# 1mishra/cbc

Hardware: AMD Instinct MI355X
Metric: Mbases/s encoded (bit-exact) on synthetic 150 bp SAM (higher is better)
Workload: dtype u32; 1 GPU; cfg2: synthetic 150 bp SAM, 10000000 reads per GPU vs a 248956422 bp uniform-ACGT contig, block-parallel encode; reads_rank0=10000000, blocks_rank0=2442, block_reads=4096, lds_bytes_per_block=15264, payload_bytes_rank0=20710203, parallelism=one GPU, no collective

## Files before the change

### cbc_amd/csrc/cbc_encode_body.h

```cpp
#ifndef CBC_ENCODE_BODY_H
#define CBC_ENCODE_BODY_H

#include <stdint.h>
#include <type_traits>
#include "../../include/cbc_gpu.h"
#include "cbc_plan.h"

#ifndef CBC_PRIO_CODER
#define CBC_PRIO_CODER 3
#define CBC_PRIO_MODEL 0
#endif
#define CBC_REC_PACK_AT 56u
#define CBC_AWORD     26u
#define CBC_M26       ((1u << 26) - 1u)
#define CBC_M25       ((1u << 25) - 1u)
#define CBC_RESCALE   (1u << 20)
#define CBC_NVARCTX   0xffffu
#define CBC_NOMEMO    0xffffffffu
#define CBC_BLOOM_LOG2 13u
#define CBC_ROLE_FUSED 0u
#define CBC_ROLE_MODEL 1u
#define CBC_ROLE_CODER 2u

#define CBC_LT_MATCH   0u
#define CBC_LT_SAMEREF 8u
#define CBC_LT_CHARS   16u

#define CBC_LDS_RLEN    0u
#define CBC_LDS_SNPS    256u
#define CBC_LDS_INDELS  512u
#define CBC_LDS_RNKEY   768u
#define CBC_LDS_RNEXC   (768u + CBC_CAP_NAME)
#define CBC_LDS_BLOOM   (768u + 2u * CBC_CAP_NAME)
#define CBC_LDS_P0      (768u + 2u * CBC_CAP_NAME + CBC_BLOOM_WORDS)
#define CBC_LDS_BATCH   CBC_PLAN_TABLE_WORDS
#ifndef CBC_BATCH_MIN
#define CBC_BATCH_MIN   40u
#endif
#define CBC_LDS_CTL     (CBC_LDS_BATCH + CBC_BATCH_SLOTS * CBC_BATCH_WORDS)
#define CBC_LDS_RING    (CBC_LDS_CTL + 8u)
#define CBC_LDS_RUN     (CBC_LDS_RING + CBC_RING_WORDS)
#define CBC_LDS_FIXED   CBC_PLAN_LDS_FIXED_WORDS

#ifdef CBC_EMU_TRACE
extern "C" void cbc_emu_trace(uint32_t read, uint32_t lo, uint32_t cnt, uint32_t n);
#endif

enum {
    CBC_PC_CODE1, CBC_PC_CODE1_REM, CBC_PC_CODE1_REM_EXACT,
    CBC_PC_QUIET, CBC_PC_QUIET_REM, CBC_PC_QUIET_REM_EXACT,
    CBC_PC_KNOWN0, CBC_PC_KNOWN0_REM,
    CBC_PC_X3, CBC_PC_X3_EXIT, CBC_PC_X3_FB_SHIFT, CBC_PC_X3_FB_REM,
    CBC_PC_SR, CBC_PC_SR_EXIT, CBC_PC_SR_FB_SHIFT, CBC_PC_SR_FB_REM,
    CBC_PC_N
};
#if defined(CBC_PATH_COUNTS) && !defined(__HIP_DEVICE_COMPILE__)
extern "C" void cbc_path_count(uint32_t what, uint32_t read);
extern "C" void cbc_path_mute(int on);
#define CBC_COUNT(what, read) cbc_path_count((what), (read))
#define CBC_COUNT_IF(cond, what, read) do { if (cond) cbc_path_count((what), (read)); } while (0)
#define CBC_COUNT_MUTE(on) cbc_path_mute(on)
#else
#define CBC_COUNT(what, read) do {} while (0)
#define CBC_COUNT_IF(cond, what, read) do {} while (0)
#define CBC_COUNT_MUTE(on) do {} while (0)
#endif

struct cbc_enc_args {
    const cbc_read_rec   *recs;
    const uint8_t        *seq;
    const uint32_t       *tok;
    const uint8_t        *names;
    const cbc_block_desc *blocks;
    const uint8_t        *ref;
    uint8_t              *out;
    cbc_block_result     *results;
    uint64_t ref_bytes, out_bytes, seq_bytes, n_tok, n_recs;
    uint32_t n_blocks, cap_pos, cap_var, names_bytes;
};

#if defined(CBC_STAMP) && defined(__HIP_DEVICE_COMPILE__)
#define CBC_T0() do { unsigned long long t_; asm volatile("s_memtime %0\n\ts_waitcnt lgkmcnt(0)" : "=s"(t_) :: "memory"); E.t_last = t_; } while (0)
#define CBC_TS(k) do { unsigned long long t_; asm volatile("s_memtime %0\n\ts_waitcnt lgkmcnt(0)" : "=s"(t_) :: "memory"); E.t_sum[k] += t_ - E.t_last; E.t_last = t_; } while (0)
#define CBC_TSM(k) do { unsigned long long t_; asm volatile("s_memtime %0\n\ts_waitcnt lgkmcnt(0)" : "=s"(t_) :: "memory"); t_sum[k] += t_ - t_last; t_last = t_; } while (0)
#elif defined(CBC_MARKS) && defined(__HIP_DEVICE_COMPILE__)
#define CBC_TSM(k) asm volatile("; ==== CBC_MARK M" #k)
#define CBC_T0() asm volatile("; ==== CBC_MARK start")
#define CBC_TS(k) asm volatile("; ==== CBC_MARK " #k)
#else
#define CBC_T0() do {} while (0)
#define CBC_TS(k) do {} while (0)
#define CBC_TSM(k) do {} while (0)
#endif

CBC_FN bool cbc_le64(uint64_t a, uint64_t b)
{
    uint32_t ah = (uint32_t)(a >> 32), al = (uint32_t)a, bh = (uint32_t)(b >> 32), bl = (uint32_t)b;
    return (ah < bh) | ((ah == bh) & (al <= bl));
}
CBC_FN bool cbc_fits64(uint64_t off, uint64_t len, uint64_t total)
{
    return cbc_le64(off, total) && cbc_le64(len, total - off);
}
CBC_FN uint32_t cbc_avail32(uint64_t total, uint32_t off)
{
    uint64_t a = total - off;
    if (!cbc_le64((uint64_t)off, total)) return 0u;
    return (uint32_t)(a >> 32) ? 0xffffffffu : (uint32_t)a;
}
CBC_FN uint32_t cbc_basepair(uint32_t c)
{
    return c == 'A' ? 0u : c == 'C' ? 1u : c == 'G' ? 2u : c == 'T' ? 3u : 4u;
}

template <class W>
struct CbcWin {
    typedef typename W::V32 V32;
    V32 w;
    CBC_MFN void clear() { w = W::splat(0u); }
    CBC_MFN void shift(uint32_t d)
    {
        if (d == 0u) return;
        if (d >= 256u) { clear(); return; }
        const V32 ln = W::lane();
        const V32 src = ln + (d >> 5);
        const V32 lo = W::lane_gather(w, src), hi = W::lane_gather(w, src + 1u);
        w = W::select(ln < 8u, W::funnel_shr(hi, lo, d & 31u), W::splat(0u));
    }
    CBC_MFN uint32_t first(uint32_t p, uint32_t rl)
    {
        uint32_t out = rl + 2u;
        if (p >= rl) return out;
        const V32 ln = W::lane();
        const uint32_t pw = p >> 5;
        const V32 a = W::select(ln == pw, w & (0xffffffffu << (p & 31u)), W::select(ln > pw, w, W::splat(0u)));
        const uint64_t hb = W::ballot(a != 0u);
        if (hb) {
            const uint32_t hl = W::ctz64(hb);
            const uint32_t pos = hl * 32u + W::ctz64((uint64_t)W::readlane(a, hl));
            if (pos < rl) out = pos - p;
        }
        return out;
    }
    CBC_MFN void set(uint32_t k)
    {
        if (k < 256u) w = w | W::select(W::lane() == (k >> 5), W::splat(1u << (k & 31u)), W::splat(0u));
    }
};

template <class W>
CBC_FN typename W::V32 cbc_small_start(uint32_t ones)
{
    typedef typename W::V32 V32;
    typedef typename W::Mask Mask;
    const V32 ln = W::lane();
    V32 sm = W::select(ln < ones, W::splat(1u), W::splat(0u));
    V32 r = (ln - CBC_LT_CHARS) >> 3, c = (ln - CBC_LT_CHARS) & 7u;
    Mask inch = (ln >= CBC_LT_CHARS) & (r < 6u) & (c < 5u);
    V32 cv = W::select(c == 4u, W::splat(1u), W::select(c == r, W::splat(0u), W::splat(8u)));
    Mask bump = ((r == 0u) & ((c == 1u) | (c == 2u))) | ((r == 1u) & ((c == 0u) | (c == 3u))) |
                ((r == 2u) & ((c == 0u) | (c == 3u))) | ((r == 3u) & ((c == 1u) | (c == 2u)));
    cv = W::select(bump, cv + 8u, cv);
    return W::select(inch, cv, sm);
}

template <class W, class = void> struct CbcHasLaneN : std::false_type {};
template <class W> struct CbcHasLaneN<W, std::void_t<decltype(&W::set_lane2_uv), decltype(&W::set_lane3)>> : std::true_type {};

template <class W, bool GEN = false>
struct CbcEnc {
    typedef typename W::V32 V32;
    typedef typename W::Mask Mask;

    typedef typename W::Uv Uv;
    Uv l, rng;
    Uv lm1;
    Uv thr0;
    CBC_MFN void set_l_forms()
    {
        lm1 = W::uv_opaque(l - 1u);
        thr0 = ((l & (1u << 24)) | (1u << 25)) - l;
    }
    static CBC_MFN bool rem_flag2(Uv tl, Uv th)
    {
#ifndef CBC_REM_OR
        if constexpr (!GEN) return W::uv_ge(tl > th ? tl : th, 0xfc000000u);
#endif
        return W::uv_ge(tl | th, 0xfc000000u);
    }
    uint32_t scale3;
    uint32_t bitpos, flushed;
    uint32_t *ring;
    uint32_t *out32; uint32_t cap_words;
    uint32_t status, nsym, fail_read, cur_read;
    V32 q_lo, q_cnt, q_n; uint32_t q_len;
    uint32_t role, batch_i; uint32_t *batch, *ctl;
    V32 b_lo, b_hi, b_n, b_fl, b_fh; uint32_t b_len, b_pos, b_stop, b_flags, seen_last;
    uint64_t b_neq;
    V32 rec_a, rec_s; uint32_t rec_n;
#ifdef CBC_STAMP
    unsigned long long t_last, t_sum[16];
#endif

    V32 small;
    V32 fkey, fexc; uint32_t fcount;
    V32 hkey, hexc; uint32_t hc0, hc1, hc2, hc3, hn0, hn1, hn2, hn3;
    uint32_t *rlen_exc, *snps_exc, *indels_exc, *rname_key, *rname_exc, *pos_val, *pos_occ, *pos_pre, *pos_idx, *var_ev, *bloom, *p0ev;
    uint32_t *runs;
    uint32_t snps_n, indels_n;
    uint32_t rn_count, rn_cap;
    uint32_t *vtab;
    uint32_t *fsp_key, *fsp_exc; uint32_t fsp_count;
    uint32_t *pos_ov_val, *pos_ov_occ; uint32_t pos_lds_cap;
    uint32_t *palpha; uint32_t pa_n0, pa_n1, pa_n2, pa_n3;
    uint32_t pos_card, cap_pos;
    uint32_t nev, nev1, cap_var;
    V32 p0cnt; uint32_t p0over;
    uint32_t L0;

    uint32_t prevPos, prevM, prevChar, win_pos;
    CbcWin<W> win;

    CBC_MFN void fail(uint32_t st) { if (status == CBC_ST_OK) { status = st; fail_read = cur_read; } }

    CBC_MFN void start_coder(uint32_t *ring_, bool pulls)
    {
        status = CBC_ST_OK; nsym = 0; fail_read = 0; cur_read = 0;
        l = W::uv(0u); set_l_forms(); rng = W::uv(CBC_M26 + 1u); scale3 = 0u; bitpos = 0; flushed = 0;
        ring = ring_;
        q_lo = W::splat(0u); q_cnt = W::splat(0u); q_n = W::splat(0u); q_len = 0;
        if (pulls) { b_lo = W::splat(0u); b_hi = W::splat(0u); b_n = W::splat(1u); b_fl = W::splat(0u); b_fh = W::splat(0u); }
        b_len = 0; b_pos = 0; b_stop = 64u; b_flags = 0; seen_last = 0; b_neq = 0;
        rec_a = W::splat(0u); rec_s = W::splat(0u); rec_n = 0;
    }
    CBC_MFN void start_handoff(uint32_t role_, uint32_t *batch_, uint32_t *ctl_) { role = role_; batch_i = 0; batch = batch_; ctl = ctl_; }
    CBC_MFN void start_models()
    {
        fkey = W::splat(0u); fexc = W::splat(0u); fcount = 0;
        hkey = W::splat(0u); hexc = W::splat(0u);
        hc0 = hc1 = hc2 = hc3 = 0; hn0 = hn1 = hn2 = hn3 = 256u;
        p0cnt = W::splat(0u); p0over = 0;
        prevPos = 0; prevM = 0; prevChar = 0; win_pos = 0;
        win_clear();
    }
    CBC_MFN void code_int(uint32_t v)
    {
        regsparse_code(hkey, hexc, 0u, 8u, hc0, hn0, 256u, 1u, v >> 24, CBC_ST_ASSERT);
        regsparse_code(hkey, hexc, 8u, 8u, hc1, hn1, 256u, 1u, (v >> 16) & 0xffu, CBC_ST_ASSERT);
        regsparse_code(hkey, hexc, 16u, 8u, hc2, hn2, 256u, 1u, (v >> 8) & 0xffu, CBC_ST_ASSERT);
        regsparse_code(hkey, hexc, 24u, 8u, hc3, hn3, 256u, 1u, v & 0xffu, CBC_ST_ASSERT);
    }

    CBC_MFN void place(const V32 &val, const V32 &len, const V32 &off, const Mask &m)
    {
        const V32 aligned = val << (W::splat(32u) - len);
        const V32 sh = off & 31u, w = (off >> 5) & (CBC_RING_WORDS - 1u);
        const Mask on = m & (len != 0u);
        W::lds_or(ring, w, aligned >> sh, on);
        W::lds_or(ring, (w + 1u) & (CBC_RING_WORDS - 1u), aligned << (W::splat(32u) - sh), on & (sh != 0u));
    }
    CBC_MFN void flush_full()
    {
        const V32 ln = W::lane();
        while ((bitpos >> 5) - flushed >= 64u) {
            const V32 idx = (ln + flushed) & (CBC_RING_WORDS - 1u);
            const V32 wv = W::load32(ring, idx, W::all(), 0u);
            if (flushed + 64u <= cap_words) W::store32(out32, ln + flushed, W::bswap_v(wv), W::all());
            else fail(CBC_ST_OUT_FULL);
            W::store32(ring, idx, W::splat(0u), W::all());
            flushed += 64u;
        }
    }
    CBC_MFN void put(uint32_t v, uint32_t n)
    {
        if (n == 0) return;
        place(W::splat(v), W::splat(n), W::splat(bitpos), W::lane() == 0u);
        bitpos += n;
        flush_full();
    }
    CBC_MFN void put_run(uint32_t bit, uint32_t n)
    {
        uint32_t pat = bit ? 0xffffffffu : 0u;
        while (n >= 32u) { put(pat, 32u); n -= 32u; }
        if (n) put(pat >> (32u - n), n);
    }
    CBC_MFN void pack(const V32 &rec_a, const V32 &rec_k3, uint32_t m)
    {
        const V32 ln = W::lane();
        const Mask in = ln < m;
        const V32 k1 = rec_a >> 26, bits = (rec_a & CBC_M26) >> ((W::splat(26u) - k1) & 31u);
        const Mask act = in & (k1 != 0u);
        const V32 k3 = W::select(in, rec_k3, W::splat(0u));
        const V32 s_in = W::scan_incl_add(k3), s_ex = s_in - k3;
        const V32 mark = W::select(act, s_ex + 1u, W::splat(0u));
// ... 817 lines not shown
            const Mask isesc = W::lane_bit(esc);
            F.p_card = cardv;
            F.p_lo = W::select(isesc, zero, c_esc + (pre0 + lt) * 10u);
            F.p_cnt = W::select(isesc, c_esc, (occ0 + eqb) * 10u);
            W::store32(pos_occ, kv, occ0 + eqa, live & (kv != 0u) & !dxbad);
        }
        {
            uint32_t carry = 0;
            const uint32_t cb = W::uni(pos_card);
            for (uint32_t b = 0; b < cb; b += 64u) {
                const V32 i = ln + b; const Mask m = (i != 0u) & (i < pos_card);
                const V32 o = W::load32(pos_occ, i, m, 0u);
                const V32 inc = W::scan_incl_add(o);
                W::store32(pos_pre, i, inc - o + carry, i < pos_card);
                carry += W::readlane(inc, 63u);
            }
        }

        st = W::select(capflag, W::splat((uint32_t)CBC_ST_CAP_FLAG), st);
        st = W::select(cappos, W::splat((uint32_t)CBC_ST_CAP_POS), st);
        st = W::select(dxbad, W::splat((uint32_t)CBC_ST_ASSERT), st);
        st = W::select(rlbad, W::splat((uint32_t)CBC_ST_ASSERT), st);
        F.st = st; F.esc = esc;
        F.bad = W::ballot(live & (st != (uint32_t)CBC_ST_OK));
    }

    CBC_MFN void var_code_dense(uint32_t ctx, uint32_t sym)
    {
        V32 ln = W::lane();
        uint32_t *row = vtab + (uint64_t)ctx * L0;
        W::list_fence();
        V32 ev[4];
        for (uint32_t q = 0; q < 4u; q++) { V32 i = ln + 64u * q; ev[q] = W::load32_list(row, i, i < L0, 0u); }
        V32 alo = W::splat(0u), aall = W::splat(0u);
        uint32_t esym = 0;
        for (uint32_t q = 0; q < 4u; q++) {
            V32 i = ln + 64u * q;
            alo = alo + W::select(i < sym, ev[q], W::splat(0u));
            aall = aall + ev[q];
            if ((sym >> 6) == q) esym = W::readlane(ev[q], sym & 63u);
        }
        const uint32_t lo = sym + W::reduce_add(alo), n = L0 + W::reduce_add(aall);
        encode(lo, 1u + esym, n);
        W::append_list(row, sym, esym + 10u);
        if (n + 10u >= CBC_RESCALE) {
            W::list_fence();
            for (uint32_t q = 0; q < 4u; q++) {
                V32 i = ln + 64u * q;
                V32 e = W::load32_list(row, i, i < L0, 0u);
                W::store32_list(row, i, (e + 1u) >> 1, i < L0);
            }
        }
    }
    CBC_MFN void var_code(uint32_t ctx, uint32_t sym)
    {
        if (ctx >= CBC_NVARCTX || sym >= L0) { fail(CBC_ST_ASSERT); return; }
        if (GEN) { var_code_dense(ctx, sym); return; }
        V32 ln = W::lane();
        uint32_t cn = 0, clo = 0, ceq = 0;
        const uint32_t key = (ctx << 8) | sym, strand1 = ctx & 1u;
        const uint32_t p0class = (((ctx >> 1) & 0x7fu) == 0u && (ctx >> 8) != 255u) ? 1u : 0u;
        uint32_t to_global = p0class ^ 1u;
        const uint32_t bkt = strand1 * 8u + ((ctx >> 8) & 7u);
        uint32_t have = 0, half_word = 0;
        if (p0class) {
            const uint32_t d = ctx >> 8, key16 = (d << 8) | sym;
            const uint32_t *arr = p0ev + bkt * CBC_P0_BUCKET_WORDS;
            have = W::readlane(p0cnt, bkt);
            const uint32_t nw = (have + 1u) >> 1;
            const V32 w = W::load32(arr, ln, ln < nw, 0xffffffffu);
            if (have & 1u) half_word = W::readlane(w, have >> 1);
            const V32 e0 = w & 0xffffu, e1 = w >> 16;
            const V32 acc = W::select((e0 >> 8) == d, W::select((e0 & 0xffu) < sym, W::splat(1u + (1u << 10)), W::splat(1u)) +
                                                       W::select(e0 == key16, W::splat(1u << 20), W::splat(0u)), W::splat(0u)) +
                            W::select((e1 >> 8) == d, W::select((e1 & 0xffu) < sym, W::splat(1u + (1u << 10)), W::splat(1u)) +
                                                       W::select(e1 == key16, W::splat(1u << 20), W::splat(0u)), W::splat(0u));
            const uint32_t tot = W::reduce_add(acc);
            cn = tot & 1023u; clo = (tot >> 10) & 1023u; ceq = tot >> 20;
            if (have >= CBC_P0_CAP) to_global = 1u;
        }
        uint32_t h1 = 0, h2 = 0, bw1 = 0, bw2 = 0, bb1 = 0, bb2 = 0;
        if ((to_global | ((p0over >> bkt) & 1u)) != 0u) {
            h1 = (ctx * 0x9E3779B1u) >> (32u - CBC_BLOOM_LOG2); h2 = (ctx * 0x85EBCA6Bu + 0x27D4EB2Fu) >> (32u - CBC_BLOOM_LOG2);
            const V32 bwv = W::load32(bloom, W::select(ln == 0u, W::splat(h1 >> 5), W::splat(h2 >> 5)), ln < 2u, 0u);
            bw1 = W::readlane(bwv, 0u); bw2 = W::readlane(bwv, 1u);
            bb1 = 1u << (h1 & 31u); bb2 = 1u << (h2 & 31u);
            if ((bw1 & bb1) && (bw2 & bb2)) {
                W::list_fence();
                const uint32_t cnt_s = strand1 ? nev1 : nev, base_s = strand1 ? cap_var - nev1 : 0u;
                const uint32_t nb = W::uni(cnt_s);
                for (uint32_t b = 0; b < nb; b += 512u) {
                    V32 ev[8];
                    for (uint32_t q = 0; q < 8u; q++) { V32 i = ln + (b + 64u * q); ev[q] = W::load32_list(var_ev, i + base_s, i < cnt_s, 0xffffffffu); }
                    for (uint32_t q = 0; q < 8u; q++) {
                        const V32 e = ev[q];
                        const uint64_t bc = W::ballot((e >> 8) == ctx);
                        if (bc) {
                            cn += W::popc64(bc);
                            clo += W::popc64(W::ballot(((e >> 8) == ctx) & ((e & 0xffu) < sym)));
                            ceq += W::popc64(W::ballot(e == key));
                        }
                    }
                }
            }
        }
        encode(sym + 10u * clo, 1u + 10u * ceq, L0 + 10u * cn);
        if (!to_global) {
            uint32_t *arr = p0ev + bkt * CBC_P0_BUCKET_WORDS;
            const uint32_t k16 = ((ctx >> 8) << 8) | sym;
            if (have & 1u) W::write_uni(arr, have >> 1, (half_word & 0xffffu) | (k16 << 16));
            else W::write_uni(arr, have >> 1, 0xffff0000u | k16);
            p0cnt = W::select(ln == bkt, p0cnt + 1u, p0cnt);
            return;
        }
        if (nev + nev1 >= cap_var) { fail(CBC_ST_CAP_VAR); return; }
        if (p0class) p0over |= 1u << bkt;
        if (!((bw1 & bb1) && (bw2 & bb2))) {
            if ((h1 >> 5) == (h2 >> 5)) W::write_uni(bloom, h1 >> 5, bw1 | bb1 | bb2);
            else { W::write_uni(bloom, h1 >> 5, bw1 | bb1); W::write_uni(bloom, h2 >> 5, bw2 | bb2); }
        }
        if (strand1) { nev1++; W::append_list(var_ev, cap_var - nev1, key); }
        else { W::append_list(var_ev, nev, key); nev++; }
    }

    CBC_MFN void win_clear() { win.clear(); }
    CBC_MFN void win_shift(uint32_t d) { win.shift(d); }
    CBC_MFN uint32_t win_first(uint32_t p, uint32_t rl) { return win.first(p, rl); }
    CBC_MFN void win_set(uint32_t k) { win.set(k); }

    struct Prep { V32 hdr0, lo, cnt; uint64_t ord; };
    CBC_MFN void prep_group(Prep &P, uint64_t neq, const V32 &r_tok, const uint32_t *tokb, uint32_t n_tok_blk)
    {
        const V32 zero = W::splat(0u);
        const Mask im = W::lane_bit(neq);
        const V32 hdr0 = W::load32(tokb, r_tok, im & (r_tok < n_tok_blk), 0u);
        const V32 hdr1 = W::load32(tokb, r_tok + 1u, im & ((r_tok + 1u) < n_tok_blk), 0u);
        const V32 n_cig = hdr0 & 0xffffu, n_md = hdr0 >> 16;
        const Mask valid = im & ((r_tok + 2u + n_cig + n_md) <= n_tok_blk) & (n_md < 1024u) &
                           ((hdr1 & 0xffffu) < 1024u) & ((hdr1 >> 16) < 1024u);
        const Mask snp_only = hdr1 == 0u;
        const V32 symv = W::select(snp_only, n_md & 0xffu, zero);
        const bool counted = snps_n + 10u * W::popc64(neq) + 10u < CBC_RESCALE;
        V32 lo_base = zero, lo_extra = zero, cntv = zero, newv = zero;
        if (counted) {
            const Mask cm = valid & (symv < L0);
            uint64_t rem = W::ballot(cm);
            while (rem) {
                const uint32_t v = W::readlane(symv, W::ctz64(rem));
                const Mask mv = cm & (symv == v);
                const uint64_t m = W::ballot(mv);
                rem &= ~m;
                uint32_t lo0, cnt0;
                dense_lookup(snps_exc, v, lo0, cnt0);
                const V32 before = W::prefix_popc(m) * 10u;
                cntv = W::select(mv, before + cnt0, cntv);
                lo_base = W::select(mv, W::splat(lo0), lo_base);
// ... 192 lines not shown
                    uint32_t k = 0, cum = 0; bool more = true;
                    for (uint32_t o = 0; o <= n_cig && E.status == CBC_ST_OK; o++) {
                        uint32_t op, len;
                        if (o < n_cig) { uint32_t t = CBC_TOK(2u + o); op = t & 15u; len = t >> 4; }
                        else { op = 99u; len = 1u; }
                        if (op == CBC_OP_M) { Mc += len; continue; }
                        if (op == CBC_OP_STAR || (op == CBC_OP_S && o == 0u)) { E.fail(CBC_ST_UNSUPPORTED); break; }
                        if (op == CBC_OP_D) {
                            if (pass == 1)
                                for (uint32_t c = 0; c < len && E.status == CBC_ST_OK; c++) {
                                    uint32_t g = Mc - prevD;
                                    if (E.q_len >= 56u) E.drain();
                                    E.var_code((p << 1) | strand, g);
                                    p += g; prevD = Mc;
                                }
                            continue;
                        }
                        for (uint32_t c = 0; c < len && E.status == CBC_ST_OK; c++) {
                            if (E.q_len >= 56u) E.drain();
                            if ((op == CBC_OP_I || op == 99u) && more && pass == 2) {
                                uint32_t limit = (op == 99u) ? rl + 1u : Mc + ins;
                                more = false;
                                while (k < n_md && E.status == CBC_ST_OK) {
                                    uint32_t t = CBC_TOK(2u + n_cig + k);
                                    uint32_t g = t >> 8;
                                    if (cum + g >= limit) { cum++; more = true; break; }
                                    if (E.q_len >= 56u) E.drain();
                                    cum += g;
                                    CBC_SNP(g, t & 0xffu, cum, p);
                                    cum++; k++;
                                }
                            }
                            if (op == 99u) break;
                            if (pass == 3) {
                                uint32_t g = Mc - prevI;
                                uint32_t base = cbc_basepair(CBC_READ_BYTE(Mc + ins));
                                E.var_code((p << 1) | strand, g);
                                p += g;
                                E.small_code(CBC_LT_CHARS + 5u * 8u, 5u, 8u, base);
                                prevI = Mc;
                            }
                            ins++;
                        }
                    }
                }
            }
            CBC_TSM(13);
#undef CBC_SNP
#undef CBC_TOK
#undef CBC_READ_BYTE
    }
};

template <class W, uint32_t ROLE>
CBC_FN void cbc_encode_stream(const cbc_enc_args &A, uint32_t blk, uint32_t *lds)
{
    const uint32_t role = ROLE;
    typedef typename W::V32 V32;
    typedef typename W::Mask Mask;
    const V32 ln = W::lane();
    const cbc_block_desc *bd = A.blocks + blk;
    CbcEnc<W> E;

    const uint64_t rec_base = bd->rec_base, seq_base = bd->seq_base, tok_base = bd->tok_base;
    const uint64_t ref_off = bd->ref_off, out_off = bd->out_off;
    const uint32_t out_cap = bd->out_cap, n_reads = bd->n_reads, name_off = bd->name_off;
    const uint32_t L0 = bd->read_length, n_tok_blk = bd->n_tok;

    E.start_coder(lds + CBC_LDS_RING, true);
    E.start_handoff(role, lds + CBC_LDS_BATCH, lds + CBC_LDS_CTL);
    if (ROLE != CBC_ROLE_FUSED) {
        if (ROLE == CBC_ROLE_MODEL) { W::write_uni(E.ctl, 0u, 0u); W::write_uni(E.ctl, 1u, 0u); W::write_uni(E.ctl, 2u, 0u); W::write_uni(E.ctl, 3u, 0u); }
        W::barrier();
    }
    const uint32_t payload_cap = bd->reserved;
    E.out32 = (uint32_t *)(A.out + out_off);
    E.cap_words = payload_cap >> 2;
    E.var_ev = (uint32_t *)(A.out + out_off + payload_cap);
    E.cap_var = payload_cap <= out_cap ? (out_cap - payload_cap) >> 2 : 0u;
    bool args_ok = cbc_fits64(out_off, out_cap, A.out_bytes) && ((out_off & 3u) == 0) && ((payload_cap & 3u) == 0) &&
                   (payload_cap <= out_cap) &&
                   cbc_fits64(rec_base, n_reads, A.n_recs) && cbc_fits64(tok_base, n_tok_blk, A.n_tok) &&
                   (L0 >= 1u && L0 <= 256u) && (name_off < A.names_bytes);
    if (!args_ok) { E.cap_words = 0; E.fail(CBC_ST_ASSERT); }
    if (n_reads > CBC_MAX_BLOCK_READS) E.fail(CBC_ST_UNSUPPORTED);

    E.L0 = L0;
    E.rlen_exc = lds + CBC_LDS_RLEN; E.snps_exc = lds + CBC_LDS_SNPS; E.indels_exc = lds + CBC_LDS_INDELS;
    E.rname_key = lds + CBC_LDS_RNKEY; E.rname_exc = lds + CBC_LDS_RNEXC;
    E.bloom = lds + CBC_LDS_BLOOM; E.p0ev = lds + CBC_LDS_P0; E.runs = lds + CBC_LDS_RUN;
    E.pos_val = lds + CBC_LDS_FIXED; E.pos_occ = E.pos_val + A.cap_pos; E.pos_pre = E.pos_occ + A.cap_pos;
    E.fsp_key = E.fsp_exc = nullptr; E.fsp_count = 0; E.pos_ov_val = E.pos_ov_occ = nullptr; E.pos_lds_cap = 0xffffffc0u; E.palpha = nullptr;
    E.pos_idx = E.pos_pre + A.cap_pos;
    E.cap_pos = A.cap_pos;
    if (ROLE != CBC_ROLE_MODEL) {
        for (uint32_t b = 0; b < CBC_POS_IDX_WORDS; b += 64u) W::store32(E.pos_idx, ln + b, W::splat(0u), W::all());
        for (uint32_t b = 0; b < CBC_RING_WORDS; b += 64u) W::store32(E.ring, ln + b, W::splat(0u), W::all());
        for (uint32_t b = 0; b < 256u; b += 64u) W::store32(E.rlen_exc, ln + b, W::splat(0u), W::all());
        W::write_uni(E.pos_val, 0u, 0xffffffffu); W::write_uni(E.pos_occ, 0u, 0u); W::write_uni(E.pos_pre, 0u, 0u);
    }
    if (ROLE != CBC_ROLE_CODER) {
        for (uint32_t b = 0; b < 512u; b += 64u) W::store32(E.snps_exc, ln + b, W::splat(0u), W::all());
        for (uint32_t b = 0; b < CBC_BLOOM_WORDS; b += 64u) W::store32(E.bloom, ln + b, W::splat(0u), W::all());
    }
    E.snps_n = L0; E.indels_n = L0;
    E.rn_count = 0; E.rn_cap = CBC_CAP_NAME; E.vtab = nullptr;
    E.pos_card = 1u;
    E.nev = 0; E.nev1 = 0;
    E.start_models();
    E.small = cbc_small_start<W>(10u);

    const uint4 *recs4 = (const uint4 *)(A.recs + rec_base);
    const uint8_t *seqb = A.seq + seq_base;
    const uint32_t *tokb = A.tok + tok_base;
    const uint8_t *refb = A.ref + ref_off;
    const uint64_t seq_avail = cbc_le64(seq_base, A.seq_bytes) ? A.seq_bytes - seq_base : 0;
    const uint64_t ref_avail = cbc_le64(ref_off, A.ref_bytes) ? A.ref_bytes - ref_off : 0;
    const uint32_t seq_lim = cbc_avail32(seq_avail, 0u), ref_lim = cbc_avail32(ref_avail, 0u);
#ifdef CBC_STAMP
    for (int i = 0; i < 16; i++) E.t_sum[i] = 0;
    CBC_T0();
#endif

    auto gen_header = [&]() {
        for (uint32_t k = 0; k < 34u && E.status == CBC_ST_OK; k++) {
            uint32_t v = (k == 0u) ? L0 : (k == 33u) ? 8u : CBC_WELL_SEED;
            E.code_int(v);
            if ((k & 7u) == 7u) E.drain();
        }
    };
    auto gen_rname = [&]() {
        for (uint32_t q = 0; E.status == CBC_ST_OK; q++) {
            uint32_t ch = (name_off + q < A.names_bytes) ? W::read_uni8(A.names, name_off + q) : 0u;
            E.rname_code(E.prevChar, ch);
            if ((q & 31u) == 31u) E.drain();
            if (ch == 0u) break;
            E.prevChar = ch;
        }
    };
    auto gen_sentinel = [&]() {
        if (E.q_len >= 56u) E.drain();
        E.cur_read = n_reads;
        E.rname_code(E.prevChar, (uint32_t)'\n');
        E.rname_code((uint32_t)'\n', 0u);
    };
    auto match_group = [&](uint32_t cn, const V32 &r_pos, const V32 &r_fl, const V32 &r_seq) -> uint64_t {
        const V32 vrl = W::select(ln < cn, r_fl >> 16, W::splat(0u));
        const V32 ro = r_pos - 1u;
        const uint32_t nd = W::uni(W::readlane(W::scan_incl_max(vrl), 63u) >> 2);
        V32 acc = W::splat(0u);
        for (uint32_t c = 0; c < nd; c += 8u) {
            V32 sv[8], rv[8];
            for (uint32_t q = 0; q < 8u; q++) {
                const uint32_t b = (c + q) * 4u;
                const Mask m = vrl >= b + 4u;
                sv[q] = W::load32_bytes(seqb + b, r_seq, m);
                rv[q] = W::load32_bytes(refb + b, ro, m);
            }
            for (uint32_t q = 0; q < 8u; q++) acc = acc | (sv[q] ^ rv[q]);
        }
        {
            const V32 tail = vrl & 3u, lb = vrl - tail;
            const Mask m = tail != 0u;
            const V32 s = W::load32_bytes(seqb, r_seq + lb, m), r = W::load32_bytes(refb, ro + lb, m);
            acc = acc | ((s ^ r) & ((W::splat(1u) << (tail * 8u)) - 1u));
        }
        return W::ballot(acc != 0u);
    };
    auto load_group = [&](uint32_t c0, V32 &r_pos, V32 &r_fl, V32 &r_seq, V32 &r_tok, bool check) -> bool {
        W::load_rec(recs4, ln + c0, (ln + c0) < n_reads, r_pos, r_fl, r_seq, r_tok);
        if (!check) return true;
        V32 vrl = r_fl >> 16;
        Mask live = (ln + c0) < n_reads;
        Mask bad = live & ((vrl == 0u) | (vrl > CBC_MAX_READ_LEN) | (r_pos == 0u) |
                           ((r_seq + vrl + 4u) > seq_lim) | ((r_pos + vrl + 3u) > ref_lim) | (r_tok >= n_tok_blk));
        uint64_t bb = W::ballot(bad);
        if (bb) { E.cur_read = c0 + W::ctz64(bb); E.fail(CBC_ST_ASSERT); return false; }
        return true;
    };

    if (ROLE == CBC_ROLE_MODEL) {
        if (CBC_PRIO_MODEL) W::prio(CBC_PRIO_MODEL);
        if (E.status == CBC_ST_OK) { gen_header(); E.seg_end(); }
        for (uint32_t c0 = 0; c0 < n_reads && E.status == CBC_ST_OK; c0 += 64u) {
            V32 r_pos, r_fl, r_seq, r_tok;
            E.cur_read = c0;
            if (E.q_len) E.publish(0u);
            uint64_t neq;
            if (!E.wait_group(c0 >> 6, neq)) { E.fail(CBC_ST_ASSERT); break; }
            load_group(c0, r_pos, r_fl, r_seq, r_tok, false);
            CBC_TS(0);
            if (c0 == 0u) { gen_rname(); E.seg_end(); }
            typename CbcEnc<W>::Prep P;
            E.prep_group(P, neq, r_tok, tokb, n_tok_blk);
            CBC_TS(14);
            uint64_t todo = neq;
            V32 nx_seq = W::splat(0u), nx_tok = W::splat(0u);
            uint32_t nx_j = 64u;
            auto prefetch = [&](uint32_t jn) {
                const uint32_t so = W::readlane(r_seq, jn), to = W::readlane(r_tok, jn), nrl = W::readlane(r_fl, jn) >> 16;
                V32 bo = ln * 4u;
                nx_seq = W::load32_bytes(seqb + so, bo, bo < nrl);
                nx_tok = W::load32(tokb + to, ln, (ln + to) < n_tok_blk, 0u);
                nx_j = jn;
            };
            auto prefetch_if_general = [&](uint64_t rest) {
                if (rest) { const uint32_t jn = W::ctz64(rest); if (!((P.ord >> jn) & 1ull)) prefetch(jn); }
            };
            typename CbcEnc<W>::Run R;
            R.pk = W::splat(0u); R.ca = R.pk; R.cb = R.pk; R.rm = 0ull; R.s = 0u; R.counted = 0u;
            while (todo && E.status == CBC_ST_OK) {
                const uint32_t j = W::ctz64(todo);
                if ((P.ord >> j) & 1ull) {
                    if (!E.run_pass(R, P, todo, r_pos, r_fl, r_seq, r_tok, tokb, seqb)) { P.ord &= ~R.rm; continue; }
                    todo &= ~R.rm;
                    prefetch_if_general(todo);
                    CBC_TS(2);
                    for (uint64_t rr = R.rm; rr && E.status == CBC_ST_OK; rr &= rr - 1ull) {
                        const uint32_t jr = W::ctz64(rr);
                        E.cur_read = c0 + jr;
                        E.run_record(R, W::readlane(P.hdr0, jr) >> 16, W::readlane(P.lo, jr), W::readlane(P.cnt, jr));
                        E.seg_end_fits();
                        CBC_TS(1);
                        if (E.q_len >= CBC_BATCH_MIN) E.drain();
                    }
                    continue;
                }
                if (nx_j != j) prefetch(j);
                todo &= todo - 1ull;
                E.cur_read = c0 + j;
                const V32 seqv = nx_seq, tokv = nx_tok;
                prefetch_if_general(todo);
                const typename CbcEnc<W>::PrepRec pr = { W::readlane(P.lo, j), W::readlane(P.cnt, j) };
                E.edits(W::readlane(r_pos, j), W::readlane(r_fl, j), W::readlane(r_tok, j), seqv, tokv, tokb, n_tok_blk, pr);
                E.seg_end_fits();
                CBC_TS(1);
                if (E.q_len >= CBC_BATCH_MIN) E.drain();
            }
        }
        if (E.status == CBC_ST_OK) { gen_sentinel(); E.seg_end(); }
#if defined(CBC_STAMP) && defined(__HIP_DEVICE_COMPILE__)
        if (E.cap_var >= 64u) for (int i = 0; i < 16; i++) {
            W::write_uni(E.var_ev + E.cap_var - 32u, 2 * i, (uint32_t)E.t_sum[i]); W::write_uni(E.var_ev + E.cap_var - 32u, 2 * i + 1, (uint32_t)(E.t_sum[i] >> 32)); }
#endif
        E.publish(CBC_BF_LAST);
        return;
    }

    const bool fused = ROLE == CBC_ROLE_FUSED;
    if (!fused) W::prio(CBC_PRIO_CODER);
    uint64_t neq_ahead = 0;
    auto look_ahead = [&](uint32_t g0) {
        V32 a_pos, a_fl, a_seq, a_tok;
        const uint32_t an = n_reads - g0 < 64u ? n_reads - g0 : 64u;
        const uint32_t saved = E.cur_read;
        CBC_TS(9);
        const bool okg = load_group(g0, a_pos, a_fl, a_seq, a_tok, true);
        neq_ahead = okg ? match_group(an, a_pos, a_fl, a_seq) : 0ull;
        E.post_group(g0 >> 6, neq_ahead, okg ? 0u : 1u);
        CBC_TS(15);
        if (okg) E.cur_read = saved;
    };
    if (!fused && n_reads != 0u && E.status == CBC_ST_OK) look_ahead(0u);
    if (E.status == CBC_ST_OK) { if (fused) { gen_header(); E.seg_end(); } else E.seg_consume(); }
    for (uint32_t c0 = 0; c0 < n_reads && E.status == CBC_ST_OK; c0 += 64u) {
        V32 r_pos, r_fl, r_seq, r_tok;
        const uint32_t cn = n_reads - c0 < 64u ? n_reads - c0 : 64u;
        E.cur_read = c0;
        uint64_t neq;
        typename CbcEnc<W>::Prep P;
        typename CbcEnc<W>::Run R;
        R.pk = W::splat(0u); R.ca = R.pk; R.cb = R.pk; R.rm = 0ull; R.s = 0u; R.counted = 0u;
        if (fused) {
            if (!load_group(c0, r_pos, r_fl, r_seq, r_tok, true)) break;
            neq = match_group(cn, r_pos, r_fl, r_seq);
            E.prep_group(P, neq, r_tok, tokb, n_tok_blk);
        } else {
            neq = neq_ahead;
            if (c0 + 64u < n_reads) look_ahead(c0 + 64u);
            if (E.status != CBC_ST_OK) break;
            load_group(c0, r_pos, r_fl, r_seq, r_tok, false);
        }
        typename CbcEnc<W>::Fixed F;
        E.fixed_group(F, c0, cn, r_pos, r_fl, neq);
        const V32 rdv = ln + c0;
        const V32 sr_hi = rdv * 10u - 9u, sr_n = rdv * 10u + 2u;
        const V32 sr_fh = CBC_FRAC(sr_hi, sr_n);
        const V32 t_hi = rdv * 10u + 1u, t_n = rdv * 10u + 255u;
        const V32 t_fh = CBC_FRAC(t_hi, t_n);
        const V32 rl_hi = F.rl_lo + F.rl_cnt;
        const V32 rl_fl = CBC_FRAC(F.rl_lo, t_n), rl_fh = CBC_FRAC(rl_hi, t_n);
        const V32 p_n = (F.p_card - 1u) * 10u + rdv * 10u + 1u, p_hi = F.p_lo + F.p_cnt;
        const V32 p_fl = CBC_FRAC(F.p_lo, p_n), p_fh = CBC_FRAC(p_hi, p_n);
        const V32 fl_n = rdv * 8u + 65536u, fl_hi = F.fl_lo + F.fl_cnt;
        const V32 fl_fl = CBC_FRAC(F.fl_lo, fl_n), fl_fh = CBC_FRAC(fl_hi, fl_n);
        const V32 m_hi = F.m_lo + F.m_cnt;
        const V32 m_fl = CBC_FRAC(F.m_lo, F.m_n), m_fh = CBC_FRAC(m_hi, F.m_n);

#define CBC_LZ(expr) [&]() -> uint32_t { return (expr); }
        auto code_record = [&](uint32_t j, auto first, auto esc) {
            const uint32_t r = c0 + j;
            E.cur_read = r;
            E.room(8u);
            const uint32_t tn = 255u + 10u * r;
            if (decltype(first)::value) {
                E.encode(1u, 1u, 2u); E.drain_q();
                if (fused) { gen_rname(); E.seg_end(); } else E.seg_consume();
            }
            if (decltype(first)::value) {
                const uint32_t tf = W::readlane(t_fh, j);
                E.step_fixed_quiet(CBC_LZ(W::readlane(F.rl_lo, j)), CBC_LZ(W::readlane(rl_hi, j)), CBC_LZ(tn), W::readlane(rl_fl, j), W::readlane(rl_fh, j));
                E.step_known0(CBC_LZ(W::readlane(t_hi, j)), CBC_LZ(tn), tf);
                E.step_known0(CBC_LZ(W::readlane(t_hi, j)), CBC_LZ(tn), tf);
                E.step_known0(CBC_LZ(W::readlane(t_hi, j)), CBC_LZ(tn), tf);
            } else {
                E.step_sameref_rl0(CBC_LZ(W::readlane(sr_hi, j)), CBC_LZ(10u * r + 2u), W::readlane(sr_fh, j),
                                   CBC_LZ(W::readlane(F.rl_lo, j)), CBC_LZ(W::readlane(rl_hi, j)), CBC_LZ(tn), W::readlane(rl_fl, j), W::readlane(rl_fh, j));
                E.step_known0_x3(CBC_LZ(W::readlane(t_hi, j)), CBC_LZ(tn), W::readlane(t_fh, j));
            }
            E.step_fixed(CBC_LZ(W::readlane(F.p_lo, j)), CBC_LZ(W::readlane(p_hi, j)), CBC_LZ(W::readlane(p_n, j)), W::readlane(p_fl, j), W::readlane(p_fh, j));
            if (decltype(esc)::value == 1 || (decltype(esc)::value == 2 && ((F.esc >> j) & 1ull))) {
                const uint32_t card = W::readlane(F.p_card, j);
                E.pos_alpha(W::read_uni(E.pos_val, card), card);
                E.drain_q();
            }
            E.step_fixed(CBC_LZ(W::readlane(F.fl_lo, j)), CBC_LZ(W::readlane(fl_hi, j)), CBC_LZ(65536u + 8u * r), W::readlane(fl_fl, j), W::readlane(fl_fh, j));
            E.step_fixed(CBC_LZ(W::readlane(F.m_lo, j)), CBC_LZ(W::readlane(m_hi, j)), CBC_LZ(W::readlane(F.m_n, j)), W::readlane(m_fl, j), W::readlane(m_fh, j));
            if ((neq >> j) & 1ull) {
                if (fused) {
                    if (((P.ord >> j) & 1ull) && !((R.rm >> j) & 1ull) &&
                        !E.run_pass(R, P, neq & (~0ull << j), r_pos, r_fl, r_seq, r_tok, tokb, seqb)) P.ord &= ~R.rm;
                    if ((P.ord >> j) & 1ull) E.run_record(R, W::readlane(P.hdr0, j) >> 16, W::readlane(P.lo, j), W::readlane(P.cnt, j));
                    else {
                        const uint32_t so = W::readlane(r_seq, j), to = W::readlane(r_tok, j), flw = W::readlane(r_fl, j);
                        const V32 bo = ln * 4u;
                        const V32 seqv = W::load32_bytes(seqb + so, bo, bo < (flw >> 16));
                        const V32 tokv = W::load32(tokb + to, ln, (ln + to) < n_tok_blk, 0u);
                        const typename CbcEnc<W>::PrepRec pr = { W::readlane(P.lo, j), W::readlane(P.cnt, j) };
                        E.edits(W::readlane(r_pos, j), flw, to, seqv, tokv, tokb, n_tok_blk, pr);
                    }
                    E.seg_end();
                } else E.seg_consume();
            }
        };
#undef CBC_LZ
        uint32_t jn = cn;
        if (F.bad) { const uint32_t fb = W::ctz64(F.bad); if (fb < cn) jn = fb; }
        typedef std::integral_constant<int, 0> Plain; typedef std::integral_constant<int, 1> Esc; typedef std::integral_constant<int, 2> Look;
        uint32_t j = 0;
        if (c0 == 0u && jn != 0u) { code_record(0u, std::true_type(), Look()); j = 1u; }
        while (j < jn && E.status == CBC_ST_OK) {
            const uint64_t ahead = F.esc >> j;
            uint32_t run_end = ahead ? j + W::ctz64(ahead) : jn;
            if (run_end > jn) run_end = jn;
            for (; j < run_end && E.status == CBC_ST_OK; j++) code_record(j, std::false_type(), Plain());
            if (j < jn && E.status == CBC_ST_OK) { code_record(j, std::false_type(), Esc()); j++; }
        }
        if (jn < cn && E.status == CBC_ST_OK) { E.cur_read = c0 + jn; E.fail(W::readlane(F.st, jn)); }
    }
    uint32_t nbytes = 0;
    if (E.status == CBC_ST_OK) {
        E.cur_read = n_reads;
        if (n_reads) E.encode(10u * n_reads - 9u, 11u, 10u * n_reads + 2u);
        else E.encode(1u, 1u, 2u);
        E.drain_q();
        if (fused) { gen_sentinel(); E.seg_end(); } else E.seg_consume();
    }
    if (E.status == CBC_ST_OK) { E.flush_recs(); nbytes = E.finish(); }
    if (E.status != CBC_ST_OK) nbytes = 0;
    if (!fused && E.status != CBC_ST_OK) E.abort_groups();
    if (!fused) E.pull_rest();
#if defined(CBC_STAMP) && defined(__HIP_DEVICE_COMPILE__)
    if (payload_cap >= 128u) for (int i = 0; i < 16; i++) {
        W::write_uni(E.out32, 2 * i, (uint32_t)E.t_sum[i]); W::write_uni(E.out32, 2 * i + 1, (uint32_t)(E.t_sum[i] >> 32)); }
#endif
    V32 resv = W::select(ln == 0u, W::splat(nbytes), W::select(ln == 1u, W::splat(E.status),
               W::select(ln == 2u, W::splat(E.nsym), W::splat(E.fail_read))));
    W::store32((uint32_t *)(A.results + blk), ln, resv, ln < 4u);
}

#endif
```

### cbc_amd/csrc/cbc_gpu.hip

```cpp
#include <new>
#include <time.h>
#include <dlfcn.h>
#include <rccl/rccl.h>

#include "cbc_gpu_internal.h"
#include "cbc_wave_gpu.h"
#include "cbc_encode_body.h"
#include "cbc_decode_body.h"
#include "cbc_stream_body.h"
#include "cbc_long_body.h"
#include "cbc_covx_body.h"
#include "cbc_stats_aln_body.h"

static_assert(CbcHasLaneN<WaveGPU>::value, "WaveGPU must supply set_lane2_uv and set_lane3");

extern __shared__ uint32_t cbc_lds[];

static __device__ __forceinline__ void cbc_encode_block(const cbc_enc_args &A)
{
    uint32_t blk = blockIdx.x;
    if (blk >= A.n_blocks) return;
    const uint32_t wid = (uint32_t)__builtin_amdgcn_readfirstlane((int)(threadIdx.x >> 6));
    if (wid == 0u) cbc_encode_stream<WaveGPU, CBC_ROLE_MODEL>(A, blk, cbc_lds);
    else cbc_encode_stream<WaveGPU, CBC_ROLE_CODER>(A, blk, cbc_lds);
}

__global__ void __launch_bounds__(128) __attribute__((amdgpu_waves_per_eu(5)))
cbc_encode_blocks_kernel(cbc_enc_args A) { cbc_encode_block(A); }

__global__ void __launch_bounds__(128) __attribute__((amdgpu_waves_per_eu(6)))
cbc_encode_blocks_kernel_w6(cbc_enc_args A) { cbc_encode_block(A); }

__global__ void __launch_bounds__(64)
cbc_decode_blocks_kernel(cbc_dec_args A)
{
    uint32_t blk = blockIdx.x;
    if (blk >= A.n_blocks) return;
    cbc_decode_stream<WaveGPU>(A, blk, cbc_lds);
}

__global__ void __launch_bounds__(64)
cbc_decode_blocks_span_kernel(cbc_dec_args A, uint32_t smax)
{
    uint32_t blk = blockIdx.x;
    if (blk >= A.n_blocks) return;
    cbc_decode_stream<WaveGPU, true>(A, blk, cbc_lds, smax);
}

__global__ void __launch_bounds__(64)
cbc_decode_blocks_edits_kernel(cbc_dec_args A, uint32_t smax, cbc_dec_edits E)
{
    uint32_t blk = blockIdx.x;
    if (blk >= A.n_blocks) return;
    cbc_decode_stream<WaveGPU, true, true>(A, blk, cbc_lds, smax, &E);
}

__global__ void __launch_bounds__(64)
cbc_encode_whole_kernel(cbc_stream_args A)
{
    const uint32_t n_streams = A.per_segment ? A.n_segs : 1u;
    for (uint32_t s = blockIdx.x; s < n_streams; s += gridDim.x) {
        if (s != blockIdx.x) {
            uint4 *t = (uint4 *)(A.vtab + (uint64_t)blockIdx.x * CBC_VTAB_WORDS);
            for (uint64_t i = threadIdx.x; i < CBC_VTAB_WORDS / 4; i += 64) t[i] = make_uint4(0, 0, 0, 0);
            __threadfence();
        }
        cbc_encode_whole<WaveGPU>(A, s, blockIdx.x, cbc_lds);
    }
}

__global__ void __launch_bounds__(64)
cbc_decode_whole_kernel(cbc_dstream_args A) { cbc_decode_whole<WaveGPU>(A, cbc_lds); }

#ifndef CBC_LONG_ENC_WAVES
#define CBC_LONG_ENC_WAVES 8
#endif
__global__ void __launch_bounds__(192) __attribute__((amdgpu_waves_per_eu(CBC_LONG_ENC_WAVES)))
cbc_long_encode_kernel(cbc_long_args A)
{
    if (blockIdx.x >= A.n_blocks) return;
    const uint32_t wid = (uint32_t)__builtin_amdgcn_readfirstlane((int)(threadIdx.x >> 6));
    if (wid == 0u) cbc_long_encode<WaveGPU, CBC_ROLE_MODEL>(A, blockIdx.x, cbc_lds);
    else if (wid == 1u) cbc_long_encode<WaveGPU, CBC_ROLE_CODER>(A, blockIdx.x, cbc_lds);
    else cbc_long_encode<WaveGPU, CBC_ROLE_WALKER>(A, blockIdx.x, cbc_lds);
// ... 1861 lines not shown
```

Before: 240,600 Mbases/s.

## Add register-resident hot variant context for the most frequent var_code key

Adds a dedicated register-held count table (two V32 pairs of packed 16-bit counts per strand) for the single hottest variant context (L0+2), so var_code for that context skips the LDS p0 bucket search, bloom lookup and global scan. The counts are prefix-summed with a wave reduction to derive the cumulative frequency. It also adds host-side counters and extra timing slots for profiling. The cost is extra VGPR pressure in the encode kernel (w5 variant only by default), which could hurt occupancy, and it relies on coding matching the original model exactly.

```diff
diff --git a/cbc_amd/csrc/cbc_encode_body.h b/cbc_amd/csrc/cbc_encode_body.h
--- a/cbc_amd/csrc/cbc_encode_body.h
+++ b/cbc_amd/csrc/cbc_encode_body.h
@@ -66,6 +66,31 @@
 #define CBC_COUNT_MUTE(on) do {} while (0)
 #endif
 
+enum {
+    CBC_VC_CALLS, CBC_VC_P0,
+    CBC_VC_HOT,
+    CBC_VC_FULL,
+    CBC_VC_BLOOM,
+    CBC_VC_SCAN, CBC_VC_SCAN_P0,
+    CBC_VC_N
+};
+#if defined(CBC_VAR_COUNTS) && !defined(__HIP_DEVICE_COMPILE__)
+extern "C" void cbc_var_count(uint32_t what, uint32_t strand);
+extern "C" void cbc_var_block(uint32_t blk);
+extern "C" int cbc_var_hot_off(void);
+#define CBC_VCOUNT(what, strand) cbc_var_count((what), (strand))
+#define CBC_VBLOCK(blk) cbc_var_block(blk)
+#define CBC_VAR_HOT_OFF() (cbc_var_hot_off() != 0)
+#else
+#define CBC_VCOUNT(what, strand) do {} while (0)
+#define CBC_VBLOCK(blk) do {} while (0)
+#define CBC_VAR_HOT_OFF() false
+#endif
+
+#ifndef CBC_HOT_CTX
+#define CBC_HOT_CTX 1
+#endif
+
 struct cbc_enc_args {
     const cbc_read_rec   *recs;
     const uint8_t        *seq;
@@ -83,15 +108,22 @@
 #define CBC_T0() do { unsigned long long t_; asm volatile("s_memtime %0\n\ts_waitcnt lgkmcnt(0)" : "=s"(t_) :: "memory"); E.t_last = t_; } while (0)
 #define CBC_TS(k) do { unsigned long long t_; asm volatile("s_memtime %0\n\ts_waitcnt lgkmcnt(0)" : "=s"(t_) :: "memory"); E.t_sum[k] += t_ - E.t_last; E.t_last = t_; } while (0)
 #define CBC_TSM(k) do { unsigned long long t_; asm volatile("s_memtime %0\n\ts_waitcnt lgkmcnt(0)" : "=s"(t_) :: "memory"); t_sum[k] += t_ - t_last; t_last = t_; } while (0)
+#define CBC_TN0(v) unsigned long long v; asm volatile("s_memtime %0\n\ts_waitcnt lgkmcnt(0)" : "=s"(v) :: "memory")
+#define CBC_TN(v, k) do { unsigned long long t_; asm volatile("s_memtime %0\n\ts_waitcnt lgkmcnt(0)" : "=s"(t_) :: "memory"); t_sum[k] += t_ - v; } while (0)
 #elif defined(CBC_MARKS) && defined(__HIP_DEVICE_COMPILE__)
 #define CBC_TSM(k) asm volatile("; ==== CBC_MARK M" #k)
+#define CBC_TN0(v) asm volatile("; ==== CBC_MARK N0")
+#define CBC_TN(v, k) asm volatile("; ==== CBC_MARK N" #k)
 #define CBC_T0() asm volatile("; ==== CBC_MARK start")
 #define CBC_TS(k) asm volatile("; ==== CBC_MARK " #k)
 #else
 #define CBC_T0() do {} while (0)
 #define CBC_TS(k) do {} while (0)
 #define CBC_TSM(k) do {} while (0)
-#endif
+#define CBC_TN0(v) do {} while (0)
+#define CBC_TN(v, k) do {} while (0)
+#endif
+#define CBC_STAMP_SLOTS 18
 
 CBC_FN bool cbc_le64(uint64_t a, uint64_t b)
 {
@@ -167,8 +199,9 @@
 template <class W, class = void> struct CbcHasLaneN : std::false_type {};
 template <class W> struct CbcHasLaneN<W, std::void_t<decltype(&W::set_lane2_uv), decltype(&W::set_lane3)>> : std::true_type {};
 
-template <class W, bool GEN = false>
+template <class W, bool GEN = false, bool HOT = false>
 struct CbcEnc {
+    static_assert(!(GEN && HOT), "the hot var context belongs to the block kernels");
     typedef typename W::V32 V32;
     typedef typename W::Mask Mask;
 
@@ -199,7 +232,7 @@
     uint64_t b_neq;
     V32 rec_a, rec_s; uint32_t rec_n;
 #ifdef CBC_STAMP
-    unsigned long long t_last, t_sum[16];
+    unsigned long long t_last, t_sum[CBC_STAMP_SLOTS];
 #endif
 
     V32 small;
@@ -217,6 +250,7 @@
     uint32_t nev, nev1, cap_var;
     V32 p0cnt; uint32_t p0over;
     uint32_t L0;
+    V32 hot_a0, hot_b0, hot_a1, hot_b1; uint32_t hot_n0, hot_n1, hot_key;
 
     uint32_t prevPos, prevM, prevChar, win_pos;
     CbcWin<W> win;
@@ -240,6 +274,10 @@
         hkey = W::splat(0u); hexc = W::splat(0u);
         hc0 = hc1 = hc2 = hc3 = 0; hn0 = hn1 = hn2 = hn3 = 256u;
         p0cnt = W::splat(0u); p0over = 0;
+        if constexpr (HOT) {
+            hot_a0 = W::splat(0u); hot_b0 = W::splat(0u); hot_a1 = W::splat(0u); hot_b1 = W::splat(0u); hot_n0 = 0; hot_n1 = 0;
+            hot_key = (L0 + 2u <= 254u && !CBC_VAR_HOT_OFF()) ? (L0 + 2u) << 8 : 0xffffffffu;
+        }
         prevPos = 0; prevM = 0; prevChar = 0; win_pos = 0;
         win_clear();
     }
@@ -1163,10 +1201,39 @@
             }
         }
     }
+    CBC_MFN void hot_code(V32 &a, V32 &b, uint32_t &n, uint32_t sym)
+    {
+        if (n >= 0xfffeu) { fail(CBC_ST_ASSERT); return; }
+        const V32 ln = W::lane();
+        const uint32_t q = sym >> 6, r = sym & 63u;
+        const uint32_t w = (q & 2u) ? W::readlane(b, r) : W::readlane(a, r);
+        const uint32_t ceq = (w >> ((q & 1u) * 16u)) & 0xffffu;
+        const uint64_t m_all = (1ull << (16u * q)) - 1ull, m_low = (m_all << 16) | 0xffffull;
+        const Mask low = ln < r;
+        const V32 fa = a & W::select(low, W::splat((uint32_t)m_low), W::splat((uint32_t)m_all));
+        const V32 fb = b & W::select(low, W::splat((uint32_t)(m_low >> 32)), W::splat((uint32_t)(m_all >> 32)));
+        const uint32_t clo = W::reduce_add((fa & 0xffffu) + (fa >> 16) + (fb & 0xffffu) + (fb >> 16));
+        W::expect_eq((clo + ceq <= n && n < 0xffffu) ? 1u : 0u, 1u, "hot var context: a count above the use count");
+        encode(sym + 10u * clo, 1u + 10u * ceq, L0 + 10u * n);
+        const uint32_t inc = 1u << ((q & 1u) * 16u);
+        const Mask one = ln == r;
+        a = a + W::select(one, W::splat((q & 2u) ? 0u : inc), W::splat(0u));
+        b = b + W::select(one, W::splat((q & 2u) ? inc : 0u), W::splat(0u));
+        n++;
+    }
     CBC_MFN void var_code(uint32_t ctx, uint32_t sym)
     {
         if (ctx >= CBC_NVARCTX || sym >= L0) { fail(CBC_ST_ASSERT); return; }
         if (GEN) { var_code_dense(ctx, sym); return; }
+        CBC_VCOUNT(CBC_VC_CALLS, ctx & 1u);
+        if constexpr (HOT) {
+            if ((ctx & ~1u) == hot_key) {
+                CBC_VCOUNT(CBC_VC_P0, ctx & 1u); CBC_VCOUNT(CBC_VC_HOT, ctx & 1u);
+                if (ctx & 1u) hot_code(hot_a1, hot_b1, hot_n1, sym);
+                else hot_code(hot_a0, hot_b0, hot_n0, sym);
+                return;
+            }
+        }
         V32 ln = W::lane();
         uint32_t cn = 0, clo = 0, ceq = 0;
         const uint32_t key = (ctx << 8) | sym, strand1 = ctx & 1u;
@@ -1175,6 +1242,7 @@
         const uint32_t bkt = strand1 * 8u + ((ctx >> 8) & 7u);
         uint32_t have = 0, half_word = 0;
         if (p0class) {
+            CBC_VCOUNT(CBC_VC_P0, strand1);
             const uint32_t d = ctx >> 8, key16 = (d << 8) | sym;
             const uint32_t *arr = p0ev + bkt * CBC_P0_BUCKET_WORDS;
             have = W::readlane(p0cnt, bkt);
@@ -1188,15 +1256,21 @@
                                                        W::select(e1 == key16, W::splat(1u << 20), W::splat(0u)), W::splat(0u));
             const uint32_t tot = W::reduce_add(acc);
             cn = tot & 1023u; clo = (tot >> 10) & 1023u; ceq = tot >> 20;
-            if (have >= CBC_P0_CAP) to_global = 1u;
+            if (have >= CBC_P0_CAP) { to_global = 1u; CBC_VCOUNT(CBC_VC_FULL, strand1); }
         }
         uint32_t h1 = 0, h2 = 0, bw1 = 0, bw2 = 0, bb1 = 0, bb2 = 0;
         if ((to_global | ((p0over >> bkt) & 1u)) != 0u) {
+            CBC_VCOUNT(CBC_VC_BLOOM, strand1);
+            CBC_TN0(tb_);
             h1 = (ctx * 0x9E3779B1u) >> (32u - CBC_BLOOM_LOG2); h2 = (ctx * 0x85EBCA6Bu + 0x27D4EB2Fu) >> (32u - CBC_BLOOM_LOG2);
             const V32 bwv = W::load32(bloom, W::select(ln == 0u, W::splat(h1 >> 5), W::splat(h2 >> 5)), ln < 2u, 0u);
             bw1 = W::readlane(bwv, 0u); bw2 = W::readlane(bwv, 1u);
             bb1 = 1u << (h1 & 31u); bb2 = 1u << (h2 & 31u);
+            CBC_TN(tb_, 16);
             if ((bw1 & bb1) && (bw2 & bb2)) {
+                CBC_VCOUNT(CBC_VC_SCAN, strand1);
+                if (p0class) CBC_VCOUNT(CBC_VC_SCAN_P0, strand1);
+                CBC_TN0(ts_);
                 W::list_fence();
                 const uint32_t cnt_s = strand1 ? nev1 : nev, base_s = strand1 ? cap_var - nev1 : 0u;
                 const uint32_t nb = W::uni(cnt_s);
@@ -1213,6 +1287,7 @@
                         }
                     }
                 }
+                CBC_TN(ts_, 17);
             }
         }
         encode(sym + 10u * clo, 1u + 10u * ceq, L0 + 10u * cn);
@@ -1511,7 +1586,7 @@
     }
 };
 
-template <class W, uint32_t ROLE>
+template <class W, uint32_t ROLE, bool HOT = (CBC_HOT_CTX != 0)>
 CBC_FN void cbc_encode_stream(const cbc_enc_args &A, uint32_t blk, uint32_t *lds)
 {
     const uint32_t role = ROLE;
@@ -1519,7 +1594,9 @@
     typedef typename W::Mask Mask;
     const V32 ln = W::lane();
     const cbc_block_desc *bd = A.blocks + blk;
-    CbcEnc<W> E;
+    typedef CbcEnc<W, false, HOT> Enc;
+    Enc E;
+    CBC_VBLOCK(blk);
 
     const uint64_t rec_base = bd->rec_base, seq_base = bd->seq_base, tok_base = bd->tok_base;
     const uint64_t ref_off = bd->ref_off, out_off = bd->out_off;
@@ -1577,7 +1654,7 @@
     const uint64_t ref_avail = cbc_le64(ref_off, A.ref_bytes) ? A.ref_bytes - ref_off : 0;
     const uint32_t seq_lim = cbc_avail32(seq_avail, 0u), ref_lim = cbc_avail32(ref_avail, 0u);
 #ifdef CBC_STAMP
-    for (int i = 0; i < 16; i++) E.t_sum[i] = 0;
+    for (int i = 0; i < CBC_STAMP_SLOTS; i++) E.t_sum[i] = 0;
     CBC_T0();
 #endif
 
@@ -1650,7 +1727,7 @@
             load_group(c0, r_pos, r_fl, r_seq, r_tok, false);
             CBC_TS(0);
             if (c0 == 0u) { gen_rname(); E.seg_end(); }
-            typename CbcEnc<W>::Prep P;
+            typename Enc::Prep P;
             E.prep_group(P, neq, r_tok, tokb, n_tok_blk);
             CBC_TS(14);
             uint64_t todo = neq;
@@ -1666,7 +1743,7 @@
             auto prefetch_if_general = [&](uint64_t rest) {
                 if (rest) { const uint32_t jn = W::ctz64(rest); if (!((P.ord >> jn) & 1ull)) prefetch(jn); }
             };
-            typename CbcEnc<W>::Run R;
+            typename Enc::Run R;
             R.pk = W::splat(0u); R.ca = R.pk; R.cb = R.pk; R.rm = 0ull; R.s = 0u; R.counted = 0u;
             while (todo && E.status == CBC_ST_OK) {
                 const uint32_t j = W::ctz64(todo);
@@ -1690,7 +1767,7 @@
                 E.cur_read = c0 + j;
                 const V32 seqv = nx_seq, tokv = nx_tok;
                 prefetch_if_general(todo);
-                const typename CbcEnc<W>::PrepRec pr = { W::readlane(P.lo, j), W::readlane(P.cnt, j) };
+                const typename Enc::PrepRec pr = { W::readlane(P.lo, j), W::readlane(P.cnt, j) };
                 E.edits(W::readlane(r_pos, j), W::readlane(r_fl, j), W::readlane(r_tok, j), seqv, tokv, tokb, n_tok_blk, pr);
                 E.seg_end_fits();
                 CBC_TS(1);
@@ -1699,8 +1776,8 @@
         }
         if (E.status == CBC_ST_OK) { gen_sentinel(); E.seg_end(); }
 #if defined(CBC_STAMP) && defined(__HIP_DEVICE_COMPILE__)
-        if (E.cap_var >= 64u) for (int i = 0; i < 16; i++) {
-            W::write_uni(E.var_ev + E.cap_var - 32u, 2 * i, (uint32_t)E.t_sum[i]); W::write_uni(E.var_ev + E.cap_var - 32u, 2 * i + 1, (uint32_t)(E.t_sum[i] >> 32)); }
+        if (E.cap_var >= 64u) for (int i = 0; i < CBC_STAMP_SLOTS; i++) {
+            W::write_uni(E.var_ev + E.cap_var - 2u * CBC_STAMP_SLOTS, 2 * i, (uint32_t)E.t_sum[i]); W::write_uni(E.var_ev + E.cap_var - 2u * CBC_STAMP_SLOTS, 2 * i + 1, (uint32_t)(E.t_sum[i] >> 32)); }
 #endif
         E.publish(CBC_BF_LAST);
         return;
@@ -1727,8 +1804,8 @@
         const uint32_t cn = n_reads - c0 < 64u ? n_reads - c0 : 64u;
         E.cur_read = c0;
         uint64_t neq;
-        typename CbcEnc<W>::Prep P;
-        typename CbcEnc<W>::Run R;
+        typename Enc::Prep P;
+        typename Enc::Run R;
         R.pk = W::splat(0u); R.ca = R.pk; R.cb = R.pk; R.rm = 0ull; R.s = 0u; R.counted = 0u;
         if (fused) {
             if (!load_group(c0, r_pos, r_fl, r_seq, r_tok, true)) break;
@@ -1740,7 +1817,7 @@
             if (E.status != CBC_ST_OK) break;
             load_group(c0, r_pos, r_fl, r_seq, r_tok, false);
         }
-        typename CbcEnc<W>::Fixed F;
+        typename Enc::Fixed F;
         E.fixed_group(F, c0, cn, r_pos, r_fl, neq);
         const V32 rdv = ln + c0;
         const V32 sr_hi = rdv * 10u - 9u, sr_n = rdv * 10u + 2u;
@@ -1795,7 +1872,7 @@
                         const V32 bo = ln * 4u;
                         const V32 seqv = W::load32_bytes(seqb + so, bo, bo < (flw >> 16));
                         const V32 tokv = W::load32(tokb + to, ln, (ln + to) < n_tok_blk, 0u);
-                        const typename CbcEnc<W>::PrepRec pr = { W::readlane(P.lo, j), W::readlane(P.cnt, j) };
+                        const typename Enc::PrepRec pr = { W::readlane(P.lo, j), W::readlane(P.cnt, j) };
                         E.edits(W::readlane(r_pos, j), flw, to, seqv, tokv, tokb, n_tok_blk, pr);
                     }
                     E.seg_end();
@@ -1830,7 +1907,7 @@
     if (!fused && E.status != CBC_ST_OK) E.abort_groups();
     if (!fused) E.pull_rest();
 #if defined(CBC_STAMP) && defined(__HIP_DEVICE_COMPILE__)
-    if (payload_cap >= 128u) for (int i = 0; i < 16; i++) {
+    if (payload_cap >= 8u * CBC_STAMP_SLOTS) for (int i = 0; i < CBC_STAMP_SLOTS; i++) {
         W::write_uni(E.out32, 2 * i, (uint32_t)E.t_sum[i]); W::write_uni(E.out32, 2 * i + 1, (uint32_t)(E.t_sum[i] >> 32)); }
 #endif
     V32 resv = W::select(ln == 0u, W::splat(nbytes), W::select(ln == 1u, W::splat(E.status),
diff --git a/cbc_amd/csrc/cbc_gpu.hip b/cbc_amd/csrc/cbc_gpu.hip
--- a/cbc_amd/csrc/cbc_gpu.hip
+++ b/cbc_amd/csrc/cbc_gpu.hip
@@ -16,20 +16,24 @@
 
 extern __shared__ uint32_t cbc_lds[];
 
+template <bool HOT>
 static __device__ __forceinline__ void cbc_encode_block(const cbc_enc_args &A)
 {
     uint32_t blk = blockIdx.x;
     if (blk >= A.n_blocks) return;
     const uint32_t wid = (uint32_t)__builtin_amdgcn_readfirstlane((int)(threadIdx.x >> 6));
-    if (wid == 0u) cbc_encode_stream<WaveGPU, CBC_ROLE_MODEL>(A, blk, cbc_lds);
-    else cbc_encode_stream<WaveGPU, CBC_ROLE_CODER>(A, blk, cbc_lds);
-}
-
+    if (wid == 0u) cbc_encode_stream<WaveGPU, CBC_ROLE_MODEL, HOT>(A, blk, cbc_lds);
+    else cbc_encode_stream<WaveGPU, CBC_ROLE_CODER, HOT>(A, blk, cbc_lds);
+}
+
+#ifndef CBC_HOT_CTX_W6
+#define CBC_HOT_CTX_W6 0
+#endif
 __global__ void __launch_bounds__(128) __attribute__((amdgpu_waves_per_eu(5)))
-cbc_encode_blocks_kernel(cbc_enc_args A) { cbc_encode_block(A); }
+cbc_encode_blocks_kernel(cbc_enc_args A) { cbc_encode_block<CBC_HOT_CTX != 0>(A); }
 
 __global__ void __launch_bounds__(128) __attribute__((amdgpu_waves_per_eu(6)))
-cbc_encode_blocks_kernel_w6(cbc_enc_args A) { cbc_encode_block(A); }
+cbc_encode_blocks_kernel_w6(cbc_enc_args A) { cbc_encode_block<CBC_HOT_CTX_W6 != 0>(A); }
 
 __global__ void __launch_bounds__(64)
 cbc_decode_blocks_kernel(cbc_dec_args A)
```

After: 244,100 Mbases/s (median of 6 runs). 1.4% higher.
